# xuekt98/BBDM

Measured on AMD Instinct MI355X. Metric: denoise-UNet sampling steps/sec (one step = p_sample of the whole local batch: UNet forward + Brownian-Bridge update) at 256x256 pixel-space BBDM, higher is better.
Workload: dtype f32 (tile GEMMs: fp32 operands as two fp16 planes under a provable power-of-two scale, 3 fp16-MFMA terms, fp32 accumulate -- measured against fp64 MORE accurate than the six-term bf16x3 split and than the f32 MFMA; 1x1 layers (skip / qkv / proj_out) and the long-sequence attention: the same pair; sh; 1 GPU; pixel-space BBDM 256x256, batch 16, 1000-step schedule (BASELINE.json configs[1]); batch_per_gpu=16, image_size=256, schedule_steps=1000, parallelism=dp1 (independent image-pair shards)

## Files before the change

bbdm_amd/csrc/common.h:

```cpp
#pragma once
#include <hip/hip_runtime.h>
#include <stdint.h>
#include <stdio.h>
#include "../../include/bbdm_hip.h"

typedef float f32x4 __attribute__((ext_vector_type(4)));
typedef float f32x16 __attribute__((ext_vector_type(16)));

#define BBDM_WAVE 64

void bbdm_set_error(const char* fmt, ...);

enum BbdmOption { BBDM_OPT_WGRAD1X1_BF3 = 0, BBDM_OPT_WINO_IDX64, BBDM_OPT_BF3P_KERNEL, BBDM_OPT_ATTN_BF3, BBDM_OPT_ATTN_PIPE, BBDM_OPT_BF3P_PAD_ROWS, BBDM_OPT_COUNT };
int bbdm_option(int id);

#define BBDM_REQUIRE(cond, ...)            \
    do {                                   \
        if (!(cond)) {                     \
            bbdm_set_error(__VA_ARGS__);   \
            return BBDM_E_BADARG;          \
        }                                  \
    } while (0)

#define BBDM_CHECK_LAUNCH(what)                                                        \
    do {                                                                               \
        hipError_t e__ = hipGetLastError();                                            \
        if (e__ != hipSuccess) {                                                       \
            bbdm_set_error("%s: launch failed: %s", what, hipGetErrorString(e__));     \
            return BBDM_E_LAUNCH;                                                      \
        }                                                                              \
    } while (0)

constexpr int BBDM_MAX_DEVICES = 64;
static inline int bbdm_device_slot() {
    int d = 0;
    if (hipGetDevice(&d) != hipSuccess || d < 0 || d >= BBDM_MAX_DEVICES) d = 0;
    return d;
}

int bbdm_gemm_tn_impl(const float* A, int lda, size_t a_stride, const float* B, int ldb, size_t b_stride, float* C, float* bias_part,
                      int batch, long long K, int M, int N, void* stream);

namespace {
__global__ void bbdm_zero8_kernel(unsigned long long* __restrict__ p, size_t n) {
    for (size_t i = blockIdx.x * (size_t)blockDim.x + threadIdx.x; i < n; i += (size_t)gridDim.x * blockDim.x) p[i] = 0ull;
}
}
static inline void bbdm_zero_async(void* p, size_t bytes, hipStream_t st) {
    const size_t n = bytes / 8;
    if (!n) return;
    size_t blocks = (n + 255) / 256;
    if (blocks > 2048) blocks = 2048;
    hipLaunchKernelGGL(bbdm_zero8_kernel, dim3((unsigned)blocks), dim3(256), 0, st, (unsigned long long*)p, n);
}

typedef float f32x2 __attribute__((ext_vector_type(2)));
__device__ __forceinline__ void store_nt(unsigned* p, unsigned v) { __builtin_nontemporal_store(v, p); }
__device__ __forceinline__ void store_nt(float* p, float v) { __builtin_nontemporal_store(v, p); }
__device__ __forceinline__ float2 load_nt(const float2* p) {
    const f32x2 v = __builtin_nontemporal_load(reinterpret_cast<const f32x2*>(p));
    return make_float2(v.x, v.y);
}
#ifndef BBDM_KEEP_IN_BRANCH
#define BBDM_KEEP_IN_BRANCH(v) asm volatile("" : "+v"(v))
#endif
#ifndef BBDM_NT_VSTORE
#define BBDM_NT_VSTORE 0
#endif
#ifndef BBDM_NT_MLOAD
#define BBDM_NT_MLOAD 0
#endif
#ifndef BBDM_NT_MSTORE
#define BBDM_NT_MSTORE 0
#endif


static inline int cdiv(int a, int b) { return (a + b - 1) / b; }
static inline int ceil_pow2(int v) {
    int p = 1;
    while (p < v) p <<= 1;
    return p;
}
static inline int ilog2(int v) {
    int l = 0;
    while ((1 << l) < v) ++l;
    return l;
}

int bbdm_conv1x1_batched(const float* x, int ldx, size_t xz, const float* packed_w, size_t wz, float* out, int ldo, size_t oz,
                         int batch, int H, int W, int CinPad, int Cout, hipStream_t st);

extern "C" int bbdm_gemm_bf3_f32(const float* V, const void* packed_bf3, float* M, int batch, long long T, int CinPad, int Cout,
                                 void* stream);

extern "C" int bbdm_gemm_bf3p_f32(const void* a_planes, const void* b_planes, const float* bias, const float* residual, int ldr,
                                  float* M, int ldo, int batch, long long T, int CinPad, int Cout, void* stream);

int bbdm_gemm_h2p_gain_splitk(const void* a_planes, const void* b_planes, const float* bound_a, float gain_a, const float* bound_b,
                              float gain_b, float* M, int ldo, int batch, long long T, long long rows, int CinPad, int Cout, int splits,
                              void* stream);

__device__ __forceinline__ float silu_f(float v) { return v / (1.0f + expf(-v)); }
__device__ __forceinline__ float silu_fast(float v) { return v * __builtin_amdgcn_rcpf(1.0f + __expf(-v)); }
__device__ __forceinline__ float2 silu_fast2(float2 v) {
    const f32x2 x = {v.x, v.y};
    const f32x2 t = x * -0x1.715476p+0f;
    f32x2 e = {__builtin_amdgcn_exp2f(t.x), __builtin_amdgcn_exp2f(t.y)};
    e = e + 1.0f;
    const f32x2 r = {__builtin_amdgcn_rcpf(e.x), __builtin_amdgcn_rcpf(e.y)};
    const f32x2 o = x * r;
    return make_float2(o.x, o.y);
}

struct FastDiv {
    unsigned d, mul, sh;
};
static inline FastDiv fastdiv_make(unsigned d) {
    FastDiv f;
    f.d = d;
    unsigned L = 0;
    while ((1ull << L) < d) ++L;
    f.mul = (unsigned)((((1ull << L) - d) << 32) / d + 1);
    f.sh = L;
    return f;
}
__device__ __forceinline__ unsigned fastdiv(unsigned n, const FastDiv& f) { return (__umulhi(n, f.mul) + n) >> f.sh; }
```

bbdm_amd/csrc/gemm_bf3p.hip:

```cpp
#include "bf3_split.h"
#include "h2_split.h"
#include "lds_dma.h"
#include <stdlib.h>

namespace {

constexpr int KC = 16;
constexpr int UNIT = 1024;

struct Bf3pArgs {
    const unsigned char* A;
    const unsigned char* B;
    float* M;
    size_t az, bz, mz, rz;
    int T, Cout, nchunks, tilesN;
    int rgs;
    int tiles, batch, by_batch;
    int persist;
    int ksplits, kps, P;
    int ldo, ldr;
    const float* bias;
    const float* res;
    const float* hA = nullptr;
    const float* hB = nullptr;
// ... 397 lines not shown
            }
        }
    };
    float bv[2];
#pragma unroll
    for (int j = 0; j < 2; ++j) {
        const int co = cout0 + wn * 64 + j * 32 + (lane & 31);
        bv[j] = (a.bias && co < a.Cout) ? a.bias[co] : 0.f;
    }
    const unsigned lds0 = lds_address(smem);
    const unsigned aoff = (wm * 2) * NP * UNIT + (lane >> 5) * 512 + (((lane & 31) ^ ((lane >> 5) << 2)) * 16);
    const unsigned boff = (NA + (wn * 2) * NP) * UNIT + lane * 16;
    issue_b(0, smem);
    load_a(0);
    store_a(smem);
    if (n > 1) {
        issue_b(1, smem + STAGE);
        load_a(1);
        store_a(smem + STAGE);
    }
    f32x16 acc[2][2];
#pragma unroll
    for (int i = 0; i < 2; ++i)
#pragma unroll
        for (int j = 0; j < 2; ++j)
#pragma unroll
            for (int r = 0; r < 16; ++r) acc[i][j][r] = 0.f;
    frag_t fa[NP][2], fb[NP][2];
#define BF3Q_READ(dst, base, p, t) do { asm volatile("ds_read_b128 %0, %1 offset:%2" : "=v"(dst) : "v"(base), "n"(((t) * NP + (p)) * UNIT)); } while (0)
#define BF3Q_READ_A(p, base) do { BF3Q_READ(fa[p][0], base, p, 0); BF3Q_READ(fa[p][1], base, p, 1); } while (0)
#define BF3Q_READ_B(p, base) do { BF3Q_READ(fb[p][0], base, p, 0); BF3Q_READ(fb[p][1], base, p, 1); } while (0)
#define BF3Q_ALL_LANDED()                                                                                                      \
    do {                                                                                                                        \
        wait_vmcnt<0>();                                                                                                        \
        if constexpr (NP == 3)                                                                                                  \
            asm volatile("s_waitcnt lgkmcnt(0)"                                                                                 \
                         : "+v"(fa[0][0]), "+v"(fa[0][1]), "+v"(fa[1][0]), "+v"(fa[1][1]), "+v"(fa[NP - 1][0]), "+v"(fa[NP - 1][1]),  \
                           "+v"(fb[0][0]), "+v"(fb[0][1]), "+v"(fb[1][0]), "+v"(fb[1][1]), "+v"(fb[NP - 1][0]), "+v"(fb[NP - 1][1])   \
                         :: "memory");                                                                                          \
        else                                                                                                                    \
            asm volatile("s_waitcnt lgkmcnt(0)"                                                                                 \
                         : "+v"(fa[0][0]), "+v"(fa[0][1]), "+v"(fa[1][0]), "+v"(fa[1][1]),                                      \
                           "+v"(fb[0][0]), "+v"(fb[0][1]), "+v"(fb[1][0]), "+v"(fb[1][1])                                       \
                         :: "memory");                                                                                          \
    } while (0)
#define BF3Q_MFMA(A_, B_, C_)                                                                                                   \
    (NP == 3 ? __builtin_amdgcn_mfma_f32_32x32x16_bf16(BF3P_BF(A_), BF3P_BF(B_), C_, 0, 0, 0)                                    \
             : __builtin_amdgcn_mfma_f32_32x32x16_f16(__builtin_bit_cast(f16x8, A_), __builtin_bit_cast(f16x8, B_), C_, 0, 0, 0))
#define BF3Q_TERM(pa, pb)                                                                                                       \
    do {                                                                                                                        \
        acc[0][0] = BF3Q_MFMA(fa[pa][0], fb[pb][0], acc[0][0]);                                                                 \
        acc[0][1] = BF3Q_MFMA(fa[pa][0], fb[pb][1], acc[0][1]);                                                                 \
        acc[1][0] = BF3Q_MFMA(fa[pa][1], fb[pb][0], acc[1][0]);                                                                 \
        acc[1][1] = BF3Q_MFMA(fa[pa][1], fb[pb][1], acc[1][1]);                                                                 \
    } while (0)
    wait_vmcnt<0>();
    asm volatile("s_waitcnt lgkmcnt(0)" ::: "memory");
    asm volatile("" :: "v"(bv[0]), "v"(bv[1]));
    asm volatile("s_barrier" ::: "memory");
    {
        const unsigned sa = lds0 + aoff, sb = lds0 + boff;
#pragma unroll
        for (int p = 0; p < NP; ++p) { BF3Q_READ_A(p, sa); BF3Q_READ_B(p, sb); }
    }
    BF3Q_ALL_LANDED();
    asm volatile("s_barrier" ::: "memory");
    for (int chunk = 0; chunk < n; ++chunk) {
        const bool has_next = chunk + 1 < n, stage2 = chunk + 2 < n;
        const unsigned nxt = lds0 + ((chunk + 1) & 1) * STAGE;
        const unsigned sa = nxt + aoff, sb = nxt + boff;
        unsigned char* const st2 = smem + (chunk & 1) * STAGE;
        if constexpr (NP == 3) {
            __builtin_amdgcn_sched_barrier(0);
            BF3Q_TERM(1, 1);
            __builtin_amdgcn_sched_barrier(0);
            if (stage2) { issue_b(chunk + 2, st2); load_a(chunk + 2); }
            __builtin_amdgcn_sched_barrier(0);
            BF3Q_TERM(0, 2);
            __builtin_amdgcn_sched_barrier(0);
            if (has_next) BF3Q_READ_B(2, sb);
            __builtin_amdgcn_sched_barrier(0);
            BF3Q_TERM(2, 0);
            __builtin_amdgcn_sched_barrier(0);
            if (has_next) BF3Q_READ_A(2, sa);
            __builtin_amdgcn_sched_barrier(0);
            BF3Q_TERM(0, 1);
            __builtin_amdgcn_sched_barrier(0);
            if (has_next) BF3Q_READ_B(1, sb);
            if (stage2) store_a(st2);
            __builtin_amdgcn_sched_barrier(0);
            BF3Q_TERM(1, 0);
            __builtin_amdgcn_sched_barrier(0);
            if (has_next) BF3Q_READ_A(1, sa);
            __builtin_amdgcn_sched_barrier(0);
            BF3Q_TERM(0, 0);
            __builtin_amdgcn_sched_barrier(0);
            if (has_next) { BF3Q_READ_A(0, sa); BF3Q_READ_B(0, sb); }
        } else {
            __builtin_amdgcn_sched_barrier(0);
            BF3Q_TERM(0, 1);
            __builtin_amdgcn_sched_barrier(0);
            if (stage2) { issue_b(chunk + 2, st2); load_a(chunk + 2); }
            if (has_next) BF3Q_READ_B(1, sb);
            __builtin_amdgcn_sched_barrier(0);
            BF3Q_TERM(0, 0);
            __builtin_amdgcn_sched_barrier(0);
            if (has_next) BF3Q_READ_A(0, sa);
            if (stage2) store_a(st2);
            __builtin_amdgcn_sched_barrier(0);
            BF3Q_TERM(1, 0);
            __builtin_amdgcn_sched_barrier(0);
            if (has_next) { BF3Q_READ_A(1, sa); BF3Q_READ_B(0, sb); }
        }
        BF3Q_ALL_LANDED();
        asm volatile("s_barrier" ::: "memory");
    }
#undef BF3Q_TERM
#undef BF3Q_MFMA
#undef BF3Q_ALL_LANDED
#undef BF3Q_READ_B
#undef BF3Q_READ_A
#undef BF3Q_READ
#pragma unroll
    for (int i = 0; i < 2; ++i)
#pragma unroll
        for (int r0 = 0; r0 < 16; r0 += 8) {
            float rv[8][2];
            if (RES) {
#pragma unroll
                for (int rr = 0; rr < 8; ++rr) {
                    const int r = r0 + rr;
                    const int row = min(row0 + wm * 64 + i * 32 + (r & 3) + 8 * (r >> 2) + 4 * (lane >> 5), a.T - 1);
#pragma unroll
                    for (int j = 0; j < 2; ++j) {
                        const int co = cout0 + wn * 64 + j * 32 + (lane & 31);
                        rv[rr][j] = co < a.Cout ? res[(size_t)row * a.ldr + co] : 0.f;
                    }
                }
            }
#pragma unroll
            for (int rr = 0; rr < 8; ++rr) {
                const int r = r0 + rr;
                const int row = row0 + wm * 64 + i * 32 + (r & 3) + 8 * (r >> 2) + 4 * (lane >> 5);
                float* dst = M + (size_t)row * a.ldo;
#pragma unroll
                for (int j = 0; j < 2; ++j) {
                    const int co = cout0 + wn * 64 + j * 32 + (lane & 31);
                    float v = (NP == 2 ? acc[i][j][r] * descale : acc[i][j][r]) + bv[j];
                    if (RES) v += rv[rr][j];
                    if (co < a.Cout && row < a.T) dst[co] = v;
                }
            }
        }
}

template <bool RES, int NS, int NP = 3>
__global__ void __launch_bounds__(256, 1) gemm_bf3s_kernel(const Bf3pArgs a, const float* __restrict__ Af, int lda) {
    extern __shared__ __attribute__((aligned(16))) unsigned char smem[];
    constexpr int CH = 4;
    constexpr int ASTAGE = 64 * CH * KC * 4;
    constexpr int BSTAGE = 2 * CH * NP * UNIT;
    constexpr int STAGE = ASTAGE + BSTAGE;
    constexpr int KA = ASTAGE / UNIT / 4, KB = BSTAGE / UNIT / 4;
    const int tid = threadIdx.x, lane = tid & 63;
    const unsigned lane16 = lane * 16;
    const int wave = __builtin_amdgcn_readfirstlane(tid >> 6);
    const int wm = wave >> 1, wn = wave & 1;
    const int tilesM = (a.T + 63) / 64, tilesN = (a.Cout + 63) / 64;
    int m_tile, n_tile;
    if (a.by_batch) {
        const int L = (int)blockIdx.x, j = L >> 3;
        n_tile = (L & 7) + 8 * (j / tilesM);
        m_tile = j % tilesM;
    } else {
        m_tile = (int)blockIdx.x % tilesM;
        n_tile = (int)blockIdx.x / tilesM;
    }
    if (n_tile >= tilesN) return;
    const int row0 = m_tile * 64, cout0 = n_tile * 64;
    const int n = a.nchunks / CH;
    const size_t gstride = (size_t)a.nchunks * NP * UNIT;
    const unsigned char* asrc[KA];
#pragma unroll
    for (int k = 0; k < KA; ++k) {
        const int row = (wave + 4 * k) * 4 + (lane >> 4), piece = (lane & 15) ^ (row & 15);
        const int grow = min(row0 + row, a.T - 1);
        asrc[k] = reinterpret_cast<const unsigned char*>(Af + (size_t)grow * lda) + piece * 16;
    }
    const unsigned char* bsrc[KB];
#pragma unroll
    for (int k = 0; k < KB; ++k) {
        const int u = wave + k * 4, g = u / (CH * NP), v = u % (CH * NP);
        bsrc[k] = a.B + (size_t)(n_tile * 2 + g) * gstride + (size_t)v * UNIT;
    }
    auto issue = [&](int it, unsigned char* st) {
#pragma unroll
        for (int k = 0; k < KA; ++k)
            __builtin_amdgcn_global_load_lds((const __attribute__((address_space(1))) void*)(asrc[k] + (size_t)it * (CH * KC * 4)),
                                             (__attribute__((address_space(3))) void*)(st + (wave + 4 * k) * UNIT), 16, 0, 0);
#pragma unroll
        for (int k = 0; k < KB; ++k) glds16(bsrc[k] + (size_t)it * (CH * NP * UNIT), lane16, st + ASTAGE + (wave + k * 4) * UNIT);
    };
    const int R = wm * 32 + (lane & 31), h = lane >> 5;
    const unsigned abase = (unsigned)((R >> 2) * UNIT + (R & 3) * 256);
    unsigned aoff[CH][2];
#pragma unroll
    for (int c = 0; c < CH; ++c) {
        aoff[c][0] = abase + (unsigned)((((4 * c + 2 * h) ^ (R & 15))) * 16);
        aoff[c][1] = abase + (unsigned)((((4 * c + 2 * h + 1) ^ (R & 15))) * 16);
    }
    const unsigned boff = (unsigned)(ASTAGE + (wn * CH * NP) * UNIT) + lane16;
    float ascale = 1.f, descale = 1.f;
    if constexpr (NP == 2) {
        const int ea = h2_exp_of_bound(*a.hA * a.gA), eb = h2_exp_of_bound(*a.hB * a.gB);
        ascale = __uint_as_float((unsigned)__builtin_amdgcn_readfirstlane((int)__float_as_uint(h2_pow2(ea))));
        descale = __uint_as_float((unsigned)__builtin_amdgcn_readfirstlane((int)__float_as_uint(h2_pow2(-(ea + eb)))));
    }
    float bv = 0.f;
    {
        const int co = cout0 + wn * 32 + (lane & 31);
        bv = (a.bias && co < a.Cout) ? a.bias[co] : 0.f;
    }
    f32x16 acc;
#pragma unroll
    for (int r = 0; r < 16; ++r) acc[r] = 0.f;
    auto landed = [&](int it) {
        const int younger = min(NS - 2, n - 1 - it);
        if (NS >= 4 && younger >= 2) wait_vmcnt<2 * (KA + KB)>();
        else if (younger >= 1) wait_vmcnt<KA + KB>();
        else wait_vmcnt<0>();
    };
#pragma unroll
    for (int k = 0; k < NS - 1; ++k)
        if (k < n) issue(k, smem + k * STAGE);
    landed(0);
    asm volatile("" :: "v"(bv));
    asm volatile("s_barrier" ::: "memory");
    const unsigned lds0 = lds_address(smem);
    typedef float f32x4 __attribute__((ext_vector_type(4)));
    f32x4 ra[3][2];
    frag_t rb[3][NP];
    frag_t fa[2][NP];
#define BF3S_READ(set, c, base)                                                                                                 \
    do {                                                                                                                        \
        asm volatile("ds_read_b128 %0, %1" : "=v"(ra[set][0]) : "v"((base) + aoff[c][0]));                                      \
        asm volatile("ds_read_b128 %0, %1" : "=v"(ra[set][1]) : "v"((base) + aoff[c][1]));                                      \
        asm volatile("ds_read_b128 %0, %1 offset:%2" : "=v"(rb[set][0]) : "v"((base) + boff), "n"(((c) * NP + 0) * UNIT));      \
        asm volatile("ds_read_b128 %0, %1 offset:%2" : "=v"(rb[set][1]) : "v"((base) + boff), "n"(((c) * NP + 1) * UNIT));      \
        if constexpr (NP == 3)                                                                                                  \
            asm volatile("ds_read_b128 %0, %1 offset:%2" : "=v"(rb[set][NP - 1]) : "v"((base) + boff), "n"(((c) * NP + NP - 1) * UNIT)); \
    } while (0)
#define BF3S_RETURNED(set, YOUNGER)                                                                                             \
    do {                                                                                                                        \
        if constexpr (NP == 3) {                                                                                                \
            if (YOUNGER) asm volatile("s_waitcnt lgkmcnt(5)" : "+v"(ra[set][0]), "+v"(ra[set][1]), "+v"(rb[set][0]), "+v"(rb[set][1]), "+v"(rb[set][NP - 1]) :: "memory"); \
            else asm volatile("s_waitcnt lgkmcnt(0)" : "+v"(ra[set][0]), "+v"(ra[set][1]), "+v"(rb[set][0]), "+v"(rb[set][1]), "+v"(rb[set][NP - 1]) :: "memory"); \
        } else {                                                                                                                \
            if (YOUNGER) asm volatile("s_waitcnt lgkmcnt(4)" : "+v"(ra[set][0]), "+v"(ra[set][1]), "+v"(rb[set][0]), "+v"(rb[set][1]) :: "memory"); \
            else asm volatile("s_waitcnt lgkmcnt(0)" : "+v"(ra[set][0]), "+v"(ra[set][1]), "+v"(rb[set][0]), "+v"(rb[set][1]) :: "memory"); \
        }                                                                                                                       \
    } while (0)
#define BF3S_SPLIT(set, dst)                                                                                                    \
    do {                                                                                                                        \
        if constexpr (NP == 3) {                                                                                                \
            uint2 p1, p2, p3, q1, q2, q3;                                                                                       \
            split4(make_float4(ra[set][0][0], ra[set][0][1], ra[set][0][2], ra[set][0][3]), p1, p2, p3);                        \
            split4(make_float4(ra[set][1][0], ra[set][1][1], ra[set][1][2], ra[set][1][3]), q1, q2, q3);                        \
            fa[dst][0] = frag_t{(int)p1.x, (int)p1.y, (int)q1.x, (int)q1.y};                                                    \
            fa[dst][1] = frag_t{(int)p2.x, (int)p2.y, (int)q2.x, (int)q2.y};                                                    \
            fa[dst][NP - 1] = frag_t{(int)p3.x, (int)p3.y, (int)q3.x, (int)q3.y};                                               \
        } else {                                                                                                                \
            uint2 p1, p2, q1, q2;                                                                                               \
            h2_split4(make_float4(ra[set][0][0] * ascale, ra[set][0][1] * ascale, ra[set][0][2] * ascale, ra[set][0][3] * ascale), p1, p2); \
            h2_split4(make_float4(ra[set][1][0] * ascale, ra[set][1][1] * ascale, ra[set][1][2] * ascale, ra[set][1][3] * ascale), q1, q2); \
            fa[dst][0] = frag_t{(int)p1.x, (int)p1.y, (int)q1.x, (int)q1.y};                                                    \
            fa[dst][1] = frag_t{(int)p2.x, (int)p2.y, (int)q2.x, (int)q2.y};                                                    \
        }                                                                                                                       \
    } while (0)
#define BF3S_MFMAS(src, set)                                                                                                    \
    do {                                                                                                                        \
        if constexpr (NP == 3) {                                                                                                \
            _Pragma("unroll") for (int t = 0; t < 6; ++t)                                                                       \
                acc = __builtin_amdgcn_mfma_f32_32x32x16_bf16(BF3P_BF(fa[src][BF3_TA[t] % NP]), BF3P_BF(rb[set][BF3_TB[t] % NP]), acc, 0, 0, 0); \
        } else {                                                                                                                \
            acc = __builtin_amdgcn_mfma_f32_32x32x16_f16(__builtin_bit_cast(f16x8, fa[src][0]), __builtin_bit_cast(f16x8, rb[set][1]), acc, 0, 0, 0); \
            acc = __builtin_amdgcn_mfma_f32_32x32x16_f16(__builtin_bit_cast(f16x8, fa[src][0]), __builtin_bit_cast(f16x8, rb[set][0]), acc, 0, 0, 0); \
            acc = __builtin_amdgcn_mfma_f32_32x32x16_f16(__builtin_bit_cast(f16x8, fa[src][1]), __builtin_bit_cast(f16x8, rb[set][0]), acc, 0, 0, 0); \
        }                                                                                                                       \
    } while (0)
#define BF3S_INTERLEAVE()                                                                                                       \
    do {                                                                                                                        \
        _Pragma("unroll") for (int t = 0; t < (NP == 3 ? 6 : 3); ++t) {                                                         \
            __builtin_amdgcn_sched_group_barrier(0x008, 1, 0);                                                                  \
            __builtin_amdgcn_sched_group_barrier(0x002, 8, 0);                                                                  \
        }                                                                                                                       \
    } while (0)
    for (int i = 0; i < n; ++i) {
        if (i + NS - 1 < n) issue(i + NS - 1, smem + ((i + NS - 1) % NS) * STAGE);
        const unsigned st = lds0 + (unsigned)((i % NS) * STAGE);
        BF3S_READ(0, 0, st);
        BF3S_READ(1, 1, st);
        BF3S_RETURNED(0, 1);
        BF3S_SPLIT(0, 0);
        BF3S_READ(2, 2, st);
        BF3S_RETURNED(1, 1);
        __builtin_amdgcn_sched_barrier(0);
// ... 347 lines not shown
    const int CoutPad = cdiv(Cout, 128) * 128, nchunks = CinPad / KC;
    const size_t pairs = (size_t)batch * nchunks * CoutPad * (KC / 2);
    size_t blocks = (pairs + 255) / 256;
    if (blocks > 8192) blocks = 8192;
    hipLaunchKernelGGL(h2p_pack_b_kernel, dim3((unsigned)blocks), dim3(256), 0, (hipStream_t)stream, packed_f32,
                       (unsigned char*)b_planes, bound, gain, (size_t)batch * nchunks, nchunks, CoutPad);
    BBDM_CHECK_LAUNCH("gemm_h2p_pack_b");
    return BBDM_OK;
}
extern "C" int bbdm_gemm_h2p_split_rows_f32(const float* x, int ldx, void* a_planes, const float* bound, int batch, long long T,
                                            int CinPad, void* stream) {
    BBDM_REQUIRE(x && a_planes && bound && batch > 0 && T > 0 && CinPad > 0 && CinPad % KC == 0 && ldx >= CinPad && ldx % 2 == 0,
                 "gemm_h2p_split_rows: bad args");
    BBDM_REQUIRE(((uintptr_t)x & 7) == 0 && ((uintptr_t)a_planes & 15) == 0, "gemm_h2p_split_rows: alignment");
    const long long Tp = (T + 255) / 256 * 256;
    const int nchunks = CinPad / KC;
    BBDM_REQUIRE((Tp / 32) * nchunks < (1ll << 31) && batch < 65536, "gemm_h2p_split_rows: too large");
    hipLaunchKernelGGL(h2p_split_rows_kernel, dim3((unsigned)((Tp / 32) * nchunks), (unsigned)batch), dim3(256), 0,
                       (hipStream_t)stream, x, ldx, (size_t)T * ldx, (unsigned char*)a_planes, (size_t)Tp * CinPad * 4, bound, (int)T,
                       nchunks);
    BBDM_CHECK_LAUNCH("gemm_h2p_split_rows");
    return BBDM_OK;
}
extern "C" int bbdm_gemm_h2p_f32(const void* a_planes, const void* b_planes, const float* bound_a, const float* bound_b,
                                 const float* bias, const float* residual, int ldr, float* M, int ldo, int batch, long long T,
                                 int CinPad, int Cout, void* stream) {
    return bf3p_forward(a_planes, b_planes, bias, residual, ldr, M, ldo, batch, T, T, CinPad, Cout, 1, stream, 2, bound_a, bound_b);
}
extern "C" int bbdm_gemm_h2p_splitk_f32(const void* a_planes, const void* b_planes, const float* bound_a, const float* bound_b, float* M,
                                        int ldo, int batch, long long T, long long rows, int CinPad, int Cout, int splits, void* stream) {
    return bf3p_forward(a_planes, b_planes, nullptr, nullptr, 0, M, ldo, batch, T, rows, CinPad, Cout, splits, stream, 2, bound_a,
                        bound_b);
}
int bbdm_gemm_h2p_gain_splitk(const void* a_planes, const void* b_planes, const float* bound_a, float gain_a, const float* bound_b,
                              float gain_b, float* M, int ldo, int batch, long long T, long long rows, int CinPad, int Cout, int splits,
                              void* stream) {
    return bf3p_forward(a_planes, b_planes, nullptr, nullptr, 0, M, ldo, batch, T, rows, CinPad, Cout, splits, stream, 2, bound_a,
                        bound_b, gain_a, gain_b);
}

namespace {
struct TnSplit { int splits, kps, wn; };
TnSplit tn_split_for(int batch, long long K, int M, int N, int bn) {
    const int nchunks = (int)(K / KC);
    const int NPad = cdiv(N, 128) * 128;
    const long long base = (long long)batch * cdiv(M, 256) * cdiv(NPad, bn);
    long long splits = (512 + base - 1) / base;
    const long long max_splits = nchunks / 16 > 1 ? nchunks / 16 : 1;
    if (splits > max_splits) splits = max_splits;
    if (splits < 1) splits = 1;
    TnSplit t;
    t.kps = (int)((nchunks + splits - 1) / splits);
    t.splits = (nchunks + t.kps - 1) / t.kps;
    t.wn = bn / 64;
    return t;
}
TnSplit tn_split(int batch, long long K, int M, int N) {
    const int NPad = cdiv(N, 128) * 128;
    const TnSplit narrow = tn_split_for(batch, K, M, N, 128);
    if (NPad % 256) return narrow;
    const TnSplit wide = tn_split_for(batch, K, M, N, 256);
    auto cost = [&](const TnSplit& t, int bn) {
        const long long per_entry = (long long)cdiv(M, 256) * cdiv(NPad, bn), nb = (long long)batch * t.splits;
        const double rounds = nb >= 8 ? (double)((per_entry * ((nb + 7) / 8) + 31) / 32) : (double)((per_entry * nb + 255) / 256);
        return rounds * (t.kps + 4) * (bn == 256 ? 1.0 : 0.5 / 0.94);
    };
    return cost(wide, 256) <= cost(narrow, 128) ? wide : narrow;
}
}

extern "C" size_t bbdm_gemm_bf3p_tn_at_bytes(int batch, long long K, int M) {
    return (size_t)batch * (size_t)((M + 31) / 32 * 32) * (size_t)((K + 255) / 256 * 256) * 6;
}
extern "C" size_t bbdm_gemm_bf3p_tn_bt_bytes(int batch, long long K, int N) {
    return (size_t)batch * (size_t)(cdiv(N, 128) * 128) * (size_t)((K + 255) / 256 * 256) * 6;
}
extern "C" int bbdm_gemm_bf3p_tn_supported(long long K, int M, int N) {
    return K > 0 && K % 256 == 0 && K < (1ll << 31) && M > 0 && M % 32 == 0 && N > 0 && N % 4 == 0;
}
extern "C" int bbdm_gemm_bf3p_tn_splits(int batch, long long K, int M, int N) {
    if (batch <= 0 || !bbdm_gemm_bf3p_tn_supported(K, M, N)) return 0;
    return tn_split(batch, K, M, N).splits;
}

namespace {
int bf3p_tn(const void* at_planes, const void* bt_planes, float* C, int batch, long long K, int M, int N, void* stream, int np,
            const float* hA, float gA, const float* hB, float gB) {
    BBDM_REQUIRE(at_planes && bt_planes && C && batch > 0, "gemm_bf3p_tn: null pointer / bad batch");
    BBDM_REQUIRE(bbdm_gemm_bf3p_tn_supported(K, M, N), "gemm_bf3p_tn: K=%lld M=%d N=%d unsupported (K %% 256, M %% 32, N %% 4)", K, M, N);
    BBDM_REQUIRE((((uintptr_t)at_planes | (uintptr_t)bt_planes) & 15) == 0 && ((uintptr_t)C & 3) == 0, "gemm_bf3p_tn: alignment");
    BBDM_REQUIRE(np == 3 || (np == 2 && hA && hB), "gemm_h2p_tn: the fp16-pair planes need the bounds of both operands");
    const TnSplit sp = tn_split(batch, K, M, N);
    Bf3pArgs a;
    a.A = (const unsigned char*)at_planes; a.B = (const unsigned char*)bt_planes; a.M = C;
    a.T = M; a.Cout = N; a.nchunks = (int)(K / KC);
    a.rgs = (M + 31) / 32;
    const int NPad = cdiv(N, 128) * 128;
    a.tilesN = NPad / 128;
    a.az = (size_t)((M + 31) / 32 * 32) * K * 2 * np; a.bz = (size_t)NPad * K * 2 * np; a.mz = (size_t)M * N; a.rz = 0;
    a.ldo = N; a.ldr = 0; a.bias = nullptr; a.res = nullptr;
    a.ksplits = sp.splits; a.kps = sp.kps; a.P = batch;
    a.hA = hA; a.hB = hB; a.gA = gA; a.gB = gB;
    const int nb = batch * sp.splits;
    const int by_batch_env = 1;
    a.batch = nb;
    a.by_batch = (by_batch_env && nb >= 8) ? 1 : 0;
    hipStream_t st = (hipStream_t)stream;
    int rc;
    if (np == 3) rc = sp.wn == 4 ? bf3p_launch<4, 4, false>(a, nb, st) : bf3p_launch<4, 2, false>(a, nb, st);
    else rc = sp.wn == 4 ? bf3p_launch<4, 4, false, 2, 2>(a, nb, st) : bf3p_launch<4, 2, false, 2, 2>(a, nb, st);
    if (rc != BBDM_OK) return rc;
    BBDM_CHECK_LAUNCH("gemm_bf3p_tn");
    return BBDM_OK;
}
}

extern "C" int bbdm_gemm_bf3p_tn_f32(const void* at_planes, const void* bt_planes, float* C, int batch, long long K, int M, int N,
                                     void* stream) {
    return bf3p_tn(at_planes, bt_planes, C, batch, K, M, N, stream, 3, nullptr, 1.f, nullptr, 1.f);
}
extern "C" size_t bbdm_gemm_h2p_tn_at_bytes(int batch, long long K, int M) {
    return (size_t)batch * (size_t)((M + 31) / 32 * 32) * (size_t)((K + 255) / 256 * 256) * 4;
}
extern "C" size_t bbdm_gemm_h2p_tn_bt_bytes(int batch, long long K, int N) {
    return (size_t)batch * (size_t)(cdiv(N, 128) * 128) * (size_t)((K + 255) / 256 * 256) * 4;
}
extern "C" int bbdm_gemm_h2p_tn_f32(const void* at_planes, const void* bt_planes, float* C, int batch, long long K, int M, int N,
                                    const float* bound_a, float gain_a, const float* bound_b, float gain_b, void* stream) {
    return bf3p_tn(at_planes, bt_planes, C, batch, K, M, N, stream, 2, bound_a, gain_a, bound_b, gain_b);
}

namespace {
template <int WM, int WN, bool RES, int NP = 3>
int bf3q_launch(Bf3pArgs& a, const float* Af, int lda, int batch, hipStream_t st) {
    static bool attr_set_dev[BBDM_MAX_DEVICES] = {};
    bool& attr_set = attr_set_dev[bbdm_device_slot()];
    const size_t lds = 2 * (size_t)(WM * 2 * NP + WN * 2 * NP) * UNIT;
    const void* fn = reinterpret_cast<const void*>(gemm_bf3q_pipe_kernel<WM, WN, RES, NP>);
    if (!attr_set) {
        if (hipFuncSetAttribute(fn, hipFuncAttributeMaxDynamicSharedMemorySize, (int)lds) != hipSuccess) {
            bbdm_set_error("gemm_bf3q: hipFuncSetAttribute(%zu B LDS) failed", lds);
            return BBDM_E_LAUNCH;
        }
        attr_set = true;
    }
    const long long blocks = (((long long)a.T + WM * 64 - 1) / (WM * 64)) * (a.tilesN * 2 / WN);
    BBDM_REQUIRE(blocks * ((batch + 7) / 8) * 8 < (1ll << 31), "gemm_bf3q: too many tiles");
    a.tiles = (int)blocks;
    a.persist = 0;
    const dim3 grid = a.by_batch ? dim3((unsigned)(8 * blocks * ((batch + 7) / 8))) : dim3((unsigned)blocks, 1, batch);
    hipLaunchKernelGGL((gemm_bf3q_pipe_kernel<WM, WN, RES, NP>), grid, dim3(WM * WN * 64), lds, st, a, Af, lda);
    return BBDM_OK;
}
}

extern "C" int bbdm_conv1x1_bf3q_f32(const float* x, int ldx, const void* b_planes, const float* bias, const float* residual, int ldr,
                                     float* out, int ldo, long long pixels, int CinPad, int Cout, void* stream) {
    BBDM_REQUIRE(x && b_planes && out, "conv1x1_bf3q: null pointer");
    BBDM_REQUIRE(pixels > 0 && pixels < (1ll << 31) && CinPad > 0 && CinPad % KC == 0 && Cout > 0 && Cout % 4 == 0,
                 "conv1x1_bf3q: pixels=%lld CinPad=%d Cout=%d unsupported", pixels, CinPad, Cout);
    BBDM_REQUIRE(ldx % 4 == 0 && ldx >= CinPad && ldo >= Cout && (!residual || ldr >= Cout) &&
                     (((uintptr_t)x | (uintptr_t)b_planes) & 15) == 0,
                 "conv1x1_bf3q: bad pitch / alignment");
    Bf3pArgs a;
    a.A = nullptr; a.B = (const unsigned char*)b_planes; a.M = out;
    a.T = (int)pixels; a.Cout = Cout; a.nchunks = CinPad / KC;
    a.rgs = 0;
    const int CoutPad = cdiv(Cout, 128) * 128;
    a.tilesN = CoutPad / 128;
    a.az = 0; a.bz = 0; a.mz = 0; a.rz = 0;
    a.ldo = ldo; a.ldr = ldr; a.bias = bias; a.res = residual;
    a.ksplits = 1; a.kps = a.nchunks; a.P = 1; a.batch = 1; a.by_batch = 0;
    hipStream_t st = (hipStream_t)stream;
    int rc;
    if (CoutPad % 256 == 0) rc = residual ? bf3q_launch<3, 4, true>(a, x, ldx, 1, st) : bf3q_launch<3, 4, false>(a, x, ldx, 1, st);
    else rc = residual ? bf3q_launch<3, 2, true>(a, x, ldx, 1, st) : bf3q_launch<3, 2, false>(a, x, ldx, 1, st);
    if (rc != BBDM_OK) return rc;
    BBDM_CHECK_LAUNCH("conv1x1_bf3q");
    return BBDM_OK;
}

extern "C" int bbdm_conv1x1_h2q_f32(const float* x, int ldx, const void* b_planes, const float* bias, const float* residual, int ldr,
                                    float* out, int ldo, long long pixels, int CinPad, int Cout, const float* xbound, const float* wbound,
                                    void* stream) {
    BBDM_REQUIRE(x && b_planes && out && xbound && wbound, "conv1x1_h2q: null pointer");
    BBDM_REQUIRE(pixels > 0 && pixels < (1ll << 31) && CinPad > 0 && CinPad % KC == 0 && Cout > 0 && Cout % 4 == 0,
                 "conv1x1_h2q: pixels=%lld CinPad=%d Cout=%d unsupported", pixels, CinPad, Cout);
    BBDM_REQUIRE(ldx % 4 == 0 && ldx >= CinPad && ldo >= Cout && (!residual || ldr >= Cout) &&
                     (((uintptr_t)x | (uintptr_t)b_planes) & 15) == 0,
                 "conv1x1_h2q: bad pitch / alignment");
    Bf3pArgs a;
    a.A = nullptr; a.B = (const unsigned char*)b_planes; a.M = out;
    a.T = (int)pixels; a.Cout = Cout; a.nchunks = CinPad / KC;
    a.rgs = 0;
    const int CoutPad = cdiv(Cout, 128) * 128;
    a.tilesN = CoutPad / 128;
    a.az = 0; a.bz = 0; a.mz = 0; a.rz = 0;
    a.ldo = ldo; a.ldr = ldr; a.bias = bias; a.res = residual;
    a.ksplits = 1; a.kps = a.nchunks; a.P = 1; a.batch = 1; a.by_batch = 0;
    a.hA = xbound; a.hB = wbound; a.gA = 1.f;
    hipStream_t st = (hipStream_t)stream;
    int rc;
    if (CoutPad % 256 == 0) rc = residual ? bf3q_launch<4, 4, true, 2>(a, x, ldx, 1, st) : bf3q_launch<4, 4, false, 2>(a, x, ldx, 1, st);
    else rc = residual ? bf3q_launch<4, 2, true, 2>(a, x, ldx, 1, st) : bf3q_launch<4, 2, false, 2>(a, x, ldx, 1, st);
    if (rc != BBDM_OK) return rc;
    BBDM_CHECK_LAUNCH("conv1x1_h2q");
    return BBDM_OK;
}

namespace {
template <int NP>
int conv1x1_small(const float* x, int ldx, const void* b_planes, const float* bias, const float* residual, int ldr, float* out, int ldo,
                  long long pixels, int CinPad, int Cout, const float* xbound, const float* wbound, void* stream) {
    BBDM_REQUIRE(x && b_planes && out, "conv1x1_bf3s: null pointer");
    BBDM_REQUIRE(pixels > 0 && pixels < (1ll << 31) && CinPad > 0 && CinPad % 64 == 0 && Cout > 0 && Cout % 4 == 0,
                 "conv1x1_bf3s: pixels=%lld CinPad=%d Cout=%d unsupported (CinPad %% 64)", pixels, CinPad, Cout);
    BBDM_REQUIRE(ldx % 4 == 0 && ldx >= CinPad && ldo >= Cout && (!residual || ldr >= Cout) &&
                     (((uintptr_t)x | (uintptr_t)b_planes) & 15) == 0,
                 "conv1x1_bf3s: bad pitch / alignment");
    Bf3pArgs a;
    a.A = nullptr; a.B = (const unsigned char*)b_planes; a.M = out;
    a.T = (int)pixels; a.Cout = Cout; a.nchunks = CinPad / KC;
    a.rgs = 0;
    a.tilesN = cdiv(Cout, 128);
    a.az = 0; a.bz = 0; a.mz = 0; a.rz = 0;
    a.ldo = ldo; a.ldr = ldr; a.bias = bias; a.res = residual;
    a.ksplits = 1; a.kps = a.nchunks; a.P = 1; a.batch = 1; a.persist = 0; a.tiles = 0;
    a.hA = xbound; a.hB = wbound;
    const int tilesM = cdiv((int)pixels, 64), tilesN = cdiv(Cout, 64);
    a.by_batch = tilesN % 8 == 0 ? 1 : 0;
    constexpr int NS = 3;
    const size_t lds = NS * (size_t)(64 * 64 * 4 + 2 * 4 * NP * UNIT);
    static bool attr_set_dev[BBDM_MAX_DEVICES][2] = {};
    bool& attr_set = attr_set_dev[bbdm_device_slot()][residual ? 1 : 0];
    if (!attr_set) {
        const void* fn = residual ? reinterpret_cast<const void*>(gemm_bf3s_kernel<true, NS, NP>) : reinterpret_cast<const void*>(gemm_bf3s_kernel<false, NS, NP>);
        if (hipFuncSetAttribute(fn, hipFuncAttributeMaxDynamicSharedMemorySize, (int)lds) != hipSuccess) {
            bbdm_set_error("conv1x1_bf3s: hipFuncSetAttribute(%zu B LDS) failed", lds);
            return BBDM_E_LAUNCH;
        }
        attr_set = true;
    }
    BBDM_REQUIRE((long long)tilesM * tilesN < (1ll << 31), "conv1x1_bf3s: too many tiles");
    const dim3 grid((unsigned)(tilesM * tilesN));
    hipStream_t st = (hipStream_t)stream;
    if (residual) hipLaunchKernelGGL((gemm_bf3s_kernel<true, NS, NP>), grid, dim3(256), lds, st, a, x, ldx);
    else hipLaunchKernelGGL((gemm_bf3s_kernel<false, NS, NP>), grid, dim3(256), lds, st, a, x, ldx);
    BBDM_CHECK_LAUNCH("conv1x1_bf3s");
    return BBDM_OK;
}
}

extern "C" int bbdm_conv1x1_bf3s_f32(const float* x, int ldx, const void* b_planes, const float* bias, const float* residual, int ldr,
                                     float* out, int ldo, long long pixels, int CinPad, int Cout, void* stream) {
    return conv1x1_small<3>(x, ldx, b_planes, bias, residual, ldr, out, ldo, pixels, CinPad, Cout, nullptr, nullptr, stream);
}
extern "C" int bbdm_conv1x1_h2s_f32(const float* x, int ldx, const void* b_planes, const float* bias, const float* residual, int ldr,
                                    float* out, int ldo, long long pixels, int CinPad, int Cout, const float* xbound, const float* wbound,
                                    void* stream) {
    BBDM_REQUIRE(xbound && wbound, "conv1x1_h2s: null bound");
    return conv1x1_small<2>(x, ldx, b_planes, bias, residual, ldr, out, ldo, pixels, CinPad, Cout, xbound, wbound, stream);
}
```

bbdm_amd/csrc/lds_dma.h:

```cpp
#pragma once
#include "common.h"

#ifndef BBDM_WAIT_VMCNT
#define BBDM_WAIT_VMCNT(N) asm volatile("s_waitcnt vmcnt(%0)" ::"n"(N) : "memory")
#endif
template <int N>
__device__ __forceinline__ void wait_vmcnt() {
    BBDM_WAIT_VMCNT(N);
}

static __device__ __forceinline__ void glds16(const unsigned char* unit, unsigned lane16, unsigned char* lds_wave_base) {
    const unsigned long long u = (unsigned long long)(uintptr_t)unit;
    const unsigned lo = (unsigned)__builtin_amdgcn_readfirstlane((int)(unsigned)u);
    const unsigned hi = (unsigned)__builtin_amdgcn_readfirstlane((int)(unsigned)(u >> 32));
    const unsigned char* base = (const unsigned char*)(uintptr_t)(((unsigned long long)hi << 32) | lo);
    __builtin_amdgcn_global_load_lds((const __attribute__((address_space(1))) void*)(base + lane16),
                                     (__attribute__((address_space(3))) void*)lds_wave_base, 16, 0, 0);
}
```

bbdm_amd/csrc/runtime.hip:

```cpp
#include <stdarg.h>
#include <string.h>
#include "common.h"

static thread_local char g_err[512] = "";

void bbdm_set_error(const char* fmt, ...) {
    va_list ap;
    va_start(ap, fmt);
    vsnprintf(g_err, sizeof(g_err), fmt, ap);
    va_end(ap);
}

extern "C" int bbdm_version(void) { return 31; }

namespace {
struct Option { const char* name; int value; };
Option g_options[BBDM_OPT_COUNT] = {
    {"wgrad1x1_bf3", 1},
    {"wino_idx64", 0},
    {"bf3p_kernel", 6},
    {"attn_bf3", 1},
    {"attn_pipe", 2},
    {"bf3p_pad_rows", 1},
};
int option_index(const char* name) {
    if (!name) return -1;
    for (int i = 0; i < BBDM_OPT_COUNT; ++i)
        if (strcmp(name, g_options[i].name) == 0) return i;
    return -1;
}
}
int bbdm_option(int id) { return g_options[id].value; }
extern "C" int bbdm_set_option(const char* name, int value) {
    const int i = option_index(name);
    BBDM_REQUIRE(i >= 0, "bbdm_set_option: unknown option '%s'", name ? name : "(null)");
    g_options[i].value = value;
    return BBDM_OK;
}
extern "C" int bbdm_get_option(const char* name, int* value) {
    const int i = option_index(name);
    BBDM_REQUIRE(i >= 0 && value, "bbdm_get_option: unknown option '%s' / null result", name ? name : "(null)");
    *value = g_options[i].value;
    return BBDM_OK;
}
extern "C" const char* bbdm_last_error(void) { return g_err; }

namespace {
int device_cus() {
    static int cus_dev[BBDM_MAX_DEVICES] = {};
    int& cus = cus_dev[bbdm_device_slot()];
    if (!cus) {
        int dev = 0;
        hipDeviceProp_t prop;
        cus = (hipGetDevice(&dev) == hipSuccess && hipGetDeviceProperties(&prop, dev) == hipSuccess && prop.multiProcessorCount > 0)
                  ? prop.multiProcessorCount : 256;
    }
    return cus;
}
}

extern "C" int bbdm_device_cus(void) { return device_cus(); }
```

Baseline: 14.17 steps/s.

## Add 4-stage ring-pipelined persistent 1x1 fp16-pair GEMM kernel for deep-K layers

```diff
diff --git a/bbdm_amd/csrc/common.h b/bbdm_amd/csrc/common.h
--- a/bbdm_amd/csrc/common.h
+++ b/bbdm_amd/csrc/common.h
@@ -11,7 +11,7 @@
 
 void bbdm_set_error(const char* fmt, ...);
 
-enum BbdmOption { BBDM_OPT_WGRAD1X1_BF3 = 0, BBDM_OPT_WINO_IDX64, BBDM_OPT_BF3P_KERNEL, BBDM_OPT_ATTN_BF3, BBDM_OPT_ATTN_PIPE, BBDM_OPT_BF3P_PAD_ROWS, BBDM_OPT_COUNT };
+enum BbdmOption { BBDM_OPT_WGRAD1X1_BF3 = 0, BBDM_OPT_WINO_IDX64, BBDM_OPT_BF3P_KERNEL, BBDM_OPT_ATTN_BF3, BBDM_OPT_ATTN_PIPE, BBDM_OPT_BF3P_PAD_ROWS, BBDM_OPT_BF3Q_RING, BBDM_OPT_COUNT };
 int bbdm_option(int id);
 
 #define BBDM_REQUIRE(cond, ...)            \
diff --git a/bbdm_amd/csrc/gemm_bf3p.hip b/bbdm_amd/csrc/gemm_bf3p.hip
--- a/bbdm_amd/csrc/gemm_bf3p.hip
+++ b/bbdm_amd/csrc/gemm_bf3p.hip
@@ -573,6 +573,219 @@
                 }
             }
         }
+}
+
+template <bool RES>
+__global__ void __launch_bounds__(1024, 4) gemm_bf3q_ring_kernel(const Bf3pArgs a, const float* __restrict__ Af, int lda) {
+    extern __shared__ __attribute__((aligned(16))) unsigned char smem[];
+    constexpr int WM = 4, WN = 4, NP = 2, NW = WM * WN, BM = WM * 64, BN = WN * 64;
+    constexpr int NA = WM * 2 * NP, NB = WN * 2 * NP, NU = NA + NB, STAGE = NU * UNIT;
+    static_assert(NB == NW && BM * 4 == NW * 64, "one B copy per wave and one float4 of A per thread and chunk: the counted waits");
+    const int tid = threadIdx.x, lane = tid & 63;
+    const unsigned lane16 = lane * 16;
+    const int wave = __builtin_amdgcn_readfirstlane(tid >> 6);
+    const int wm = wave / WN, wn = wave % WN;
+    const int tilesN = a.tilesN * 2 / WN;
+    const size_t gstride = (size_t)a.nchunks * NP * UNIT;
+    const int n = a.nchunks;
+    const unsigned adst = (unsigned)((((tid >> 2) >> 5) * NP) * UNIT + ((tid & 3) >> 1) * 512 + ((((tid >> 2) & 31) ^ (((tid & 3) >> 1) << 2)) * 16) + (tid & 1) * 8);
+    auto thread_index = [&]() { int t = tid; BBDM_KEEP_IN_BRANCH(t); return t; };
+    const unsigned lds0 = lds_address(smem);
+    const unsigned aoff = (wm * 2) * NP * UNIT + (lane >> 5) * 512 + (((lane & 31) ^ ((lane >> 5) << 2)) * 16);
+    const unsigned boff = (NA + (wn * 2) * NP) * UNIT + lane * 16;
+    const int ea = h2_exp_of_bound(*a.hA * a.gA), eb = h2_exp_of_bound(*a.hB * a.gB);
+    const float ascale = __uint_as_float((unsigned)__builtin_amdgcn_readfirstlane((int)__float_as_uint(h2_pow2(ea))));
+    const float descale = __uint_as_float((unsigned)__builtin_amdgcn_readfirstlane((int)__float_as_uint(h2_pow2(-(ea + eb)))));
+    int row0 = 0, cout0 = 0;
+    const unsigned char* abase = nullptr;
+    unsigned avoff = 0;
+    const unsigned char* bsrc = nullptr;
+    float bv[2];
+    auto setup = [&](int L) -> bool {
+        if (L >= a.tiles) return false;
+        const int t = thread_index(), arow = t >> 2, q = t & 3, lane = t & 63;
+        const int bid = xcd_block_p(a.tiles, L, 0);
+        const int n_tile = bid % tilesN, m_tile = bid / tilesN;
+        row0 = m_tile * BM; cout0 = n_tile * BN;
+        abase = reinterpret_cast<const unsigned char*>(Af + (size_t)row0 * lda);
+        avoff = ((unsigned)(min(row0 + arow, a.T - 1) - row0) * (unsigned)lda + q * 4) * 4u;
+        bsrc = a.B + (size_t)(n_tile * (WN * 2) + wave / NP) * gstride + (wave % NP) * UNIT;
+#pragma unroll
+        for (int j = 0; j < 2; ++j) {
+            const int co = cout0 + wn * 64 + j * 32 + (lane & 31);
+            bv[j] = (a.bias && co < a.Cout) ? a.bias[co] : 0.f;
+        }
+        return true;
+    };
+    auto issue_b_to = [&](int chunk, int slot) {
+        unsigned l16 = lane16;
+        BBDM_KEEP_IN_BRANCH(l16);
+        glds16(bsrc + (size_t)chunk * (NP * UNIT), l16, smem + (slot & 3) * STAGE + (NA + wave) * UNIT);
+    };
+    auto issue_b = [&](int chunk) { issue_b_to(chunk, chunk); };
+#define BF3R_LOAD_A(dst, chunk) BBDM_LOAD16_UNTRACKED(dst, abase + (size_t)(chunk) * (KC * 4), avoff)
+    auto store_a = [&](const f32x4& v, int chunk) {
+        unsigned st = adst;
+        BBDM_KEEP_IN_BRANCH(st);
+        st += lds0 + (chunk & 3) * STAGE;
+        uint2 p1, p2;
+        h2_split4(make_float4(v.x * ascale, v.y * ascale, v.z * ascale, v.w * ascale), p1, p2);
+        BBDM_LDS_WRITE8(st, 0, p1);
+        BBDM_LDS_WRITE8(st, UNIT, p2);
+    };
+    f32x4 ax, ay, az;
+    auto request_first = [&]() {
+        BF3R_LOAD_A(ax, 0);
+        BF3R_LOAD_A(ay, min(1, n - 1));
+        BF3R_LOAD_A(az, min(2, n - 1));
+        issue_b(0);
+        issue_b_to(min(1, n - 1), 1);
+        issue_b_to(min(2, n - 1), 2);
+    };
+    frag_t fa[NP][2], fb[NP][2];
+#define BF3R_READ(dst, base, p, t) do { asm volatile("ds_read_b128 %0, %1 offset:%2" : "=v"(dst) : "v"(base), "n"(((t) * NP + (p)) * UNIT)); } while (0)
+#define BF3R_READ_A(p, base) do { BF3R_READ(fa[p][0], base, p, 0); BF3R_READ(fa[p][1], base, p, 1); } while (0)
+#define BF3R_READ_B(p, base) do { BF3R_READ(fb[p][0], base, p, 0); BF3R_READ(fb[p][1], base, p, 1); } while (0)
+#define BF3R_READS_RETURNED()                                                                                                  \
+    do {                                                                                                                        \
+        asm volatile("s_waitcnt lgkmcnt(0)"                                                                                     \
+                     : "+v"(fa[0][0]), "+v"(fa[0][1]), "+v"(fa[1][0]), "+v"(fa[1][1]),                                          \
+                       "+v"(fb[0][0]), "+v"(fb[0][1]), "+v"(fb[1][0]), "+v"(fb[1][1])                                           \
+                     :: "memory");                                                                                              \
+    } while (0)
+#define BF3R_FIRST_READS_RETURNED()                                                                                            \
+    do { asm volatile("s_waitcnt lgkmcnt(4)" : "+v"(fa[0][0]), "+v"(fa[0][1]), "+v"(fb[1][0]), "+v"(fb[1][1]) :: "memory"); } while (0)
+#define BF3R_LAST_READS_RETURNED()                                                                                             \
+    do { asm volatile("s_waitcnt lgkmcnt(0)" : "+v"(fa[1][0]), "+v"(fa[1][1]), "+v"(fb[0][0]), "+v"(fb[0][1]) :: "memory"); } while (0)
+#define BF3R_MFMA(A_, B_, C_) __builtin_amdgcn_mfma_f32_32x32x16_f16(__builtin_bit_cast(f16x8, A_), __builtin_bit_cast(f16x8, B_), C_, 0, 0, 0)
+#define BF3R_TERM(pa, pb)                                                                                                       \
+    do {                                                                                                                        \
+        acc[0][0] = BF3R_MFMA(fa[pa][0], fb[pb][0], acc[0][0]);                                                                 \
+        acc[0][1] = BF3R_MFMA(fa[pa][0], fb[pb][1], acc[0][1]);                                                                 \
+        acc[1][0] = BF3R_MFMA(fa[pa][1], fb[pb][0], acc[1][0]);                                                                 \
+        acc[1][1] = BF3R_MFMA(fa[pa][1], fb[pb][1], acc[1][1]);                                                                 \
+    } while (0)
+    int L = (int)blockIdx.x;
+    if (!setup(L)) return;
+    request_first();
+    for (;;) {
+        f32x16 acc[2][2];
+#pragma unroll
+        for (int i = 0; i < 2; ++i)
+#pragma unroll
+            for (int j = 0; j < 2; ++j)
+#pragma unroll
+                for (int r = 0; r < 16; ++r) acc[i][j][r] = 0.f;
+        asm volatile("s_waitcnt vmcnt(0)" : "+v"(ax), "+v"(ay), "+v"(az) :: "memory");
+        store_a(ax, 0);
+        store_a(ay, 1);
+        store_a(az, 2);
+        __builtin_amdgcn_s_waitcnt(0);
+        asm volatile("" :: "v"(bv[0]), "v"(bv[1]));
+        asm volatile("s_barrier" ::: "memory");
+        {
+            const unsigned sa = lds0 + aoff, sb = lds0 + boff;
+#pragma unroll
+            for (int p = 0; p < NP; ++p) { BF3R_READ_A(p, sa); BF3R_READ_B(p, sb); }
+        }
+        BF3R_READS_RETURNED();
+        asm volatile("s_barrier" ::: "memory");
+        for (int chunk = 0; chunk < n; chunk += 2) {
+            const bool has1 = chunk + 1 < n, has2 = chunk + 2 < n;
+            {
+                const unsigned nxt = lds0 + ((chunk + 1) & 3) * STAGE;
+                const unsigned sa = nxt + aoff, sb = nxt + boff;
+                __builtin_amdgcn_sched_barrier(0);
+                BF3R_TERM(0, 1);
+                __builtin_amdgcn_sched_barrier(0);
+                BF3R_LOAD_A(ax, min(chunk + 3, n - 1));
+                BF3R_LOAD_A(ay, min(chunk + 4, n - 1));
+                issue_b_to(min(chunk + 3, n - 1), chunk + 3);
+                issue_b_to(min(chunk + 4, n - 1), chunk + 4);
+                if (has1) BF3R_READ_B(1, sb);
+                __builtin_amdgcn_sched_barrier(0);
+                BF3R_TERM(0, 0);
+                __builtin_amdgcn_sched_barrier(0);
+                if (has1) BF3R_READ_A(0, sa);
+                __builtin_amdgcn_sched_barrier(0);
+                BF3R_TERM(1, 0);
+                __builtin_amdgcn_sched_barrier(0);
+                if (has1) { BF3R_READ_A(1, sa); BF3R_READ_B(0, sb); }
+            }
+            if (has1) {
+                BF3R_FIRST_READS_RETURNED();
+                const unsigned nxt = lds0 + ((chunk + 2) & 3) * STAGE;
+                const unsigned sa = nxt + aoff, sb = nxt + boff;
+                __builtin_amdgcn_sched_barrier(0);
+                BF3R_TERM(0, 1);
+                __builtin_amdgcn_sched_barrier(0);
+                BF3R_LAST_READS_RETURNED();
+                if (has2) BF3R_READ_B(1, sb);
+                asm volatile("s_waitcnt vmcnt(3)" : "+v"(ax) :: "memory");
+                store_a(ax, chunk + 3);
+                __builtin_amdgcn_sched_barrier(0);
+                BF3R_TERM(0, 0);
+                __builtin_amdgcn_sched_barrier(0);
+                if (has2) BF3R_READ_A(0, sa);
+                asm volatile("s_waitcnt vmcnt(2)" : "+v"(ay) :: "memory");
+                store_a(ay, chunk + 4);
+                __builtin_amdgcn_sched_barrier(0);
+                BF3R_TERM(1, 0);
+                __builtin_amdgcn_sched_barrier(0);
+                if (has2) { BF3R_READ_A(1, sa); BF3R_READ_B(0, sb); }
+            }
+            wait_vmcnt<0>();
+            BF3R_READS_RETURNED();
+            asm volatile("s_barrier" ::: "memory");
+        }
+        const int crow0 = row0, ccout0 = cout0;
+        const float cb0 = bv[0], cb1 = bv[1];
+        L += (int)gridDim.x;
+        const bool more = a.persist && setup(L);
+        if (more) request_first();
+        const int lane = thread_index() & 63;
+#pragma unroll
+        for (int i = 0; i < 2; ++i)
+#pragma unroll
+            for (int r0 = 0; r0 < 16; r0 += 8) {
+                float rv[8][2];
+                if (RES) {
+#pragma unroll
+                    for (int rr = 0; rr < 8; ++rr) {
+                        const int r = r0 + rr;
+                        const int row = min(crow0 + wm * 64 + i * 32 + (r & 3) + 8 * (r >> 2) + 4 * (lane >> 5), a.T - 1);
+#pragma unroll
+                        for (int j = 0; j < 2; ++j) {
+                            const int co = ccout0 + wn * 64 + j * 32 + (lane & 31);
+                            rv[rr][j] = co < a.Cout ? a.res[(size_t)row * a.ldr + co] : 0.f;
+                        }
+                    }
+                }
+#pragma unroll
+                for (int rr = 0; rr < 8; ++rr) {
+                    const int r = r0 + rr;
+                    const int row = crow0 + wm * 64 + i * 32 + (r & 3) + 8 * (r >> 2) + 4 * (lane >> 5);
+                    float* dst = a.M + (size_t)row * a.ldo;
+#pragma unroll
+                    for (int j = 0; j < 2; ++j) {
+                        const int co = ccout0 + wn * 64 + j * 32 + (lane & 31);
+                        float v = acc[i][j][r] * descale + (j ? cb1 : cb0);
+                        if (RES) v += rv[rr][j];
+                        if (co < a.Cout && row < a.T) dst[co] = v;
+                    }
+                }
+            }
+        if (!more) break;
+    }
+#undef BF3R_TERM
+#undef BF3R_MFMA
+#undef BF3R_LAST_READS_RETURNED
+#undef BF3R_FIRST_READS_RETURNED
+#undef BF3R_READS_RETURNED
+#undef BF3R_READ_B
+#undef BF3R_READ_A
+#undef BF3R_READ
+#undef BF3R_LOAD_A
 }
 
 template <bool RES, int NS, int NP = 3>
@@ -1226,6 +1439,28 @@
     hipLaunchKernelGGL((gemm_bf3q_pipe_kernel<WM, WN, RES, NP>), grid, dim3(WM * WN * 64), lds, st, a, Af, lda);
     return BBDM_OK;
 }
+
+template <bool RES>
+int bf3q_ring_launch(Bf3pArgs& a, const float* Af, int lda, bool persistent, hipStream_t st) {
+    static bool attr_set_dev[BBDM_MAX_DEVICES] = {};
+    bool& attr_set = attr_set_dev[bbdm_device_slot()];
+    const size_t lds = 4 * (size_t)(4 * 2 * 2 + 4 * 2 * 2) * UNIT;
+    if (!attr_set) {
+        if (hipFuncSetAttribute(reinterpret_cast<const void*>(gemm_bf3q_ring_kernel<RES>), hipFuncAttributeMaxDynamicSharedMemorySize,
+                                (int)lds) != hipSuccess) {
+            bbdm_set_error("gemm_bf3q_ring: hipFuncSetAttribute(%zu B LDS) failed", lds);
+            return BBDM_E_LAUNCH;
+        }
+        attr_set = true;
+    }
+    const long long blocks = (((long long)a.T + 255) / 256) * (a.tilesN / 2);
+    BBDM_REQUIRE(blocks < (1ll << 31), "gemm_bf3q_ring: too many tiles");
+    a.tiles = (int)blocks;
+    const unsigned resident = (unsigned)bbdm_device_cus() / 8 * 8;
+    a.persist = persistent && resident >= 8 && blocks > resident ? 1 : 0;
+    hipLaunchKernelGGL((gemm_bf3q_ring_kernel<RES>), dim3(a.persist ? resident : (unsigned)blocks), dim3(1024), lds, st, a, Af, lda);
+    return BBDM_OK;
+}
 }
 
 extern "C" int bbdm_conv1x1_bf3q_f32(const float* x, int ldx, const void* b_planes, const float* bias, const float* residual, int ldr,
@@ -1275,7 +1510,10 @@
     a.hA = xbound; a.hB = wbound; a.gA = 1.f;
     hipStream_t st = (hipStream_t)stream;
     int rc;
-    if (CoutPad % 256 == 0) rc = residual ? bf3q_launch<4, 4, true, 2>(a, x, ldx, 1, st) : bf3q_launch<4, 4, false, 2>(a, x, ldx, 1, st);
+    const int ring = bbdm_option(BBDM_OPT_BF3Q_RING);
+    if (CoutPad % 256 == 0 && ldx < (1 << 21) && (ring >= 2 || (ring == 1 && a.nchunks >= 16)))
+        rc = residual ? bf3q_ring_launch<true>(a, x, ldx, ring != 3, st) : bf3q_ring_launch<false>(a, x, ldx, ring != 3, st);
+    else if (CoutPad % 256 == 0) rc = residual ? bf3q_launch<4, 4, true, 2>(a, x, ldx, 1, st) : bf3q_launch<4, 4, false, 2>(a, x, ldx, 1, st);
     else rc = residual ? bf3q_launch<4, 2, true, 2>(a, x, ldx, 1, st) : bf3q_launch<4, 2, false, 2>(a, x, ldx, 1, st);
     if (rc != BBDM_OK) return rc;
     BBDM_CHECK_LAUNCH("conv1x1_h2q");
diff --git a/bbdm_amd/csrc/lds_dma.h b/bbdm_amd/csrc/lds_dma.h
--- a/bbdm_amd/csrc/lds_dma.h
+++ b/bbdm_amd/csrc/lds_dma.h
@@ -17,3 +17,22 @@
     __builtin_amdgcn_global_load_lds((const __attribute__((address_space(1))) void*)(base + lane16),
                                      (__attribute__((address_space(3))) void*)lds_wave_base, 16, 0, 0);
 }
+
+#ifndef BBDM_LOAD16_UNTRACKED
+#define BBDM_LOAD16_UNTRACKED(dst, base, voff)                                                                                 \
+    do {                                                                                                                        \
+        const unsigned long long u__ = (unsigned long long)(uintptr_t)(base);                                                  \
+        const unsigned lo__ = (unsigned)__builtin_amdgcn_readfirstlane((int)(unsigned)u__);                                    \
+        const unsigned hi__ = (unsigned)__builtin_amdgcn_readfirstlane((int)(unsigned)(u__ >> 32));                            \
+        asm volatile("global_load_dwordx4 %0, %1, %2" : "=v"(dst) : "v"(voff), "s"(((unsigned long long)hi__ << 32) | lo__) : "memory"); \
+    } while (0)
+#endif
+
+#ifndef BBDM_LDS_WRITE8
+typedef unsigned bbdm_u32x2 __attribute__((ext_vector_type(2)));
+#define BBDM_LDS_WRITE8(addr, off, v)                                                                                          \
+    do {                                                                                                                        \
+        const bbdm_u32x2 v__ = {(v).x, (v).y};                                                                                  \
+        asm volatile("ds_write_b64 %0, %1 offset:%2" ::"v"(addr), "v"(v__), "n"(off) : "memory");                              \
+    } while (0)
+#endif
diff --git a/bbdm_amd/csrc/runtime.hip b/bbdm_amd/csrc/runtime.hip
--- a/bbdm_amd/csrc/runtime.hip
+++ b/bbdm_amd/csrc/runtime.hip
@@ -22,6 +22,7 @@
     {"attn_bf3", 1},
     {"attn_pipe", 2},
     {"bf3p_pad_rows", 1},
+    {"bf3q_ring", 1},
 };
 int option_index(const char* name) {
     if (!name) return -1;
```

After: 14.22 steps/s, median of 2. No clear change (+0.4%).
